# linto-ai/whisper-timestamped

Measured on NVIDIA H100. Metric: audio-sec/s (RTF) large-v3 1h synthetic @1/2/4/8 H100; DTW GB/s vs HBM peak, higher is better.
Workload: dtype bf16x3 tensor-core GEMMs (float32-accurate), f32 elsewhere, f64 DTW accumulate

## Files before the change

whisper-timestamped_b200/csrc/gemm_tc.cu:

```cuda
#include <cuda_bf16.h>

#include "sm90.cuh"

namespace wts {

constexpr int BM = 128, BN = 128, BK = 64;
constexpr int TILE_BYTES = BM * BK * 2;
constexpr int STAGES = 3;
constexpr int STAGE_BYTES = 4 * TILE_BYTES;
constexpr int PT_THREADS = 384;
constexpr int PT_PRODUCER_REGS = 40, PT_CONSUMER_REGS = 232;
static_assert(128 * PT_PRODUCER_REGS + 256 * PT_CONSUMER_REGS <= 65536, "setmaxnreg plan exceeds the register file");
constexpr int GROUP_M = 8;
constexpr int GT_SMEM = STAGES * STAGE_BYTES + 256 + 1024;
constexpr int PART_LD = BN + 4;

template <int WG>
struct SplitTraits {
    static constexpr int A_BYTES = 64 * WG * BK * 2;
    static constexpr int STAGE_BYTES = 2 * A_BYTES + 2 * TILE_BYTES;
    static constexpr int STAGES = WG == 1 ? 4 : 3;
    static constexpr int THREADS = 128 * WG + 32;
    static_assert(STAGES * STAGE_BYTES + 256 + 1024 == GT_SMEM, "a 192 KB ring: the persistent kernel's shared memory");
    static_assert(64 * WG * PART_LD * 4 <= STAGES * STAGE_BYTES, "the partial tile lives in the operand ring");
};

__device__ __forceinline__ float gelu_erf_tc(float v) { return 0.5f * v * (1.0f + erff(v * 0.70710678118654752440f)); }

struct TcArgs {
    WtsGemm g;
    int a_has_bo, a_has_bi, b_has_bo, b_has_bi;
    int split_k;
    int pair_stores;
};

__device__ __forceinline__ int64_t out_offset(const WtsGemm& g, int m, int n, int64_t ld)
{
    return g.head_dim > 0 ? (int64_t)(n / g.head_dim) * g.head_stride + (int64_t)m * ld + (n % g.head_dim)
                          : (int64_t)m * ld + n;
}

__device__ __forceinline__ void store_one(const WtsGemm& g, int m, int n, float t, float* of, __nv_bfloat16* ob)
{
    if (of) of[out_offset(g, m, n, g.ldc)] = t;
    if (ob) {
        const __nv_bfloat16 hi = __float2bfloat16_rn(t);
        __nv_bfloat16* d = ob + out_offset(g, m, n, g.ldo);
        d[0] = hi;
        d[g.o_plane] = __float2bfloat16_rn(t - __bfloat162float(hi));
    }
}

__device__ __forceinline__ float2 pair_values(const WtsGemm& g, int n, bool two, float v0, float v1, float bias_m, const float* res)
{
    float t0 = g.alpha * v0, t1 = g.alpha * v1;
    if (g.bias) {
        t0 += g.bias_on_m ? bias_m : g.bias[n];
        if (two) t1 += g.bias_on_m ? bias_m : g.bias[n + 1];
    }
    if (g.act == 1) { t0 = gelu_erf_tc(t0); t1 = gelu_erf_tc(t1); }
    if (res) { t0 += res[n]; if (two) t1 += res[n + 1]; }
    return make_float2(t0, t1);
}

__device__ __forceinline__ void store_pair_sb16(__nv_bfloat16* dh, int64_t plane, float t0, float t1)
{
    const __nv_bfloat162 hi = __floats2bfloat162_rn(t0, t1);
    const __nv_bfloat162 lo = __floats2bfloat162_rn(t0 - __low2float(hi), t1 - __high2float(hi));
    *reinterpret_cast<__nv_bfloat162*>(dh) = hi;
    *reinterpret_cast<__nv_bfloat162*>(dh + plane) = lo;
}

__device__ __forceinline__ void epilogue_pair(const WtsGemm& g, int m, int n, float v0, float v1, float bias_m,
                                              const float* res, float* of, __nv_bfloat16* ob)
{
    const bool two = n + 1 < g.N;
    const float2 t = pair_values(g, n, two, v0, v1, bias_m, res);
    const float t0 = t.x, t1 = t.y;
    const bool same_head = g.head_dim == 0 || (n % g.head_dim) + 1 < g.head_dim;
    if (!(two && same_head)) {
        store_one(g, m, n, t0, of, ob);
        if (two) store_one(g, m, n + 1, t1, of, ob);
        return;
    }
    if (of) {
        float* d = of + out_offset(g, m, n, g.ldc);
        if ((reinterpret_cast<uintptr_t>(d) & 7) == 0) *reinterpret_cast<float2*>(d) = make_float2(t0, t1);
        else { d[0] = t0; d[1] = t1; }
    }
    if (ob) {
        __nv_bfloat16* dh = ob + out_offset(g, m, n, g.ldo);
        __nv_bfloat16* dl = dh + g.o_plane;
        if (((reinterpret_cast<uintptr_t>(dh) | reinterpret_cast<uintptr_t>(dl)) & 3) == 0) {
            store_pair_sb16(dh, g.o_plane, t0, t1);
        } else {
            const __nv_bfloat162 hi = __floats2bfloat162_rn(t0, t1);
            const __nv_bfloat162 lo = __floats2bfloat162_rn(t0 - __low2float(hi), t1 - __high2float(hi));
            dh[0] = hi.x; dh[1] = hi.y; dl[0] = lo.x; dl[1] = lo.y;
        }
    }
}

template <bool PAIRS>
__device__ __forceinline__ void epilogue_frag64(const WtsGemm& g, int zo, int zi, int m_base, int n0, const float (&acc)[64])
{
    const int lane = threadIdx.x & 31;
    const int cl = 2 * (lane & 3);
    float* of = g.out_f32 ? g.out_f32 + (int64_t)zo * g.c_bo + (int64_t)zi * g.c_bi : nullptr;
    __nv_bfloat16* ob = g.out_sb16 ? reinterpret_cast<__nv_bfloat16*>(g.out_sb16) + (int64_t)zo * g.o_bo + (int64_t)zi * g.o_bi : nullptr;
#pragma unroll
    for (int i = 0; i < 2; ++i) {
        const int m = m_base + (lane >> 2) + 8 * i;
        if (m >= g.M || (g.row_mask && g.row_mask[m] == 0)) continue;
        const float* res = g.residual ? g.residual + (int64_t)zo * g.r_bo + (int64_t)zi * g.r_bi + (int64_t)m * g.ldr : nullptr;
        const float bias_m = (g.bias && g.bias_on_m) ? g.bias[m] : 0.f;
#pragma unroll
        for (int j = 0; j < 16; ++j) {
            const int n = n0 + cl + 8 * j;
            if (PAIRS) {
                const float2 t = pair_values(g, n, true, acc[4 * j + 2 * i], acc[4 * j + 2 * i + 1], bias_m, res);
                if (of) *reinterpret_cast<float2*>(of + out_offset(g, m, n, g.ldc)) = t;
                if (ob) store_pair_sb16(ob + out_offset(g, m, n, g.ldo), g.o_plane, t.x, t.y);
            } else if (n < g.N) {
                epilogue_pair(g, m, n, acc[4 * j + 2 * i], acc[4 * j + 2 * i + 1], bias_m, res, of, ob);
            }
        }
    }
}

__device__ __forceinline__ void split_epilogue_one(const WtsGemm& g, int m, int n, const float (&x)[8], float bias_n)
{
    float t = 0.f;
#pragma unroll
    for (int s = 0; s < 8; ++s) t += x[s];
    t = g.alpha * t + (g.bias ? (g.bias_on_m ? g.bias[m] : bias_n) : 0.f);
    if (g.act == 1) t = gelu_erf_tc(t);
    if (g.residual) t += g.residual[(int64_t)m * g.ldr + n];
    store_one(g, m, n, t, g.out_f32, reinterpret_cast<__nv_bfloat16*>(g.out_sb16));
}

__device__ __forceinline__ void named_bar_sync(int id, int n) { asm volatile("bar.sync %0, %1;" ::"r"(id), "r"(n) : "memory"); }
__device__ __forceinline__ void named_bar_arrive(int id, int n) { asm volatile("bar.arrive %0, %1;" ::"r"(id), "r"(n) : "memory"); }

struct TileCoord { int m0, n0, zo, zi; };

__device__ __forceinline__ TileCoord tile_coord(const WtsGemm& g, int t, int tiles_m, int tiles_n)
{
    const int per_batch = tiles_m * tiles_n;
    const int z = t / per_batch;
    int r = t - z * per_batch;
    const int span = GROUP_M * tiles_n;
    const int grp = r / span;
    const int m_first = grp * GROUP_M;
    const int gm = min(GROUP_M, tiles_m - m_first);
    r -= grp * span;
    TileCoord c;
    c.m0 = (m_first + r % gm) * BM;
    c.n0 = (r / gm) * BN;
    c.zo = z / g.batch_inner;
    c.zi = z - c.zo * g.batch_inner;
    return c;
}

__global__ void __launch_bounds__(PT_THREADS, 1)
gemm_tc_kernel(const __grid_constant__ CUtensorMap tmA, const __grid_constant__ CUtensorMap tmB, const TcArgs args)
{
    extern __shared__ unsigned char smem_raw[];
    const WtsGemm& g = args.g;
    const uint32_t base = (smem_addr(smem_raw) + 1023u) & ~1023u;
    const uint32_t bar = base + STAGES * STAGE_BYTES;
    const int wg = threadIdx.x >> 7, warp = (threadIdx.x >> 5) & 3, lane = threadIdx.x & 31;
    const int tiles_n = (g.N + BN - 1) / BN, tiles_m = (g.M + BM - 1) / BM;
    const int tiles = tiles_m * tiles_n * g.batch_outer * g.batch_inner;
    const int nkb = (g.K + BK - 1) / BK;
    pdl_launch();

    if (threadIdx.x == 0) {
        asm volatile("prefetch.tensormap [%0];" ::"l"(&tmA) : "memory");
        asm volatile("prefetch.tensormap [%0];" ::"l"(&tmB) : "memory");
        for (int s = 0; s < STAGES; ++s) { mbar_init(bar + 8 * s, 1); mbar_init(bar + 32 + 8 * s, 4); }
        asm volatile("fence.mbarrier_init.release.cluster;" ::: "memory");
    }
    __syncthreads();
    pdl_wait();

    if (wg == 0) {
        asm volatile("setmaxnreg.dec.sync.aligned.u32 %0;" ::"n"(PT_PRODUCER_REGS));
        if (warp == 0 && lane == 0) {
            int p = 0;
            for (int t = blockIdx.x; t < tiles; t += gridDim.x) {
                const TileCoord tc = tile_coord(g, t, tiles_m, tiles_n);
                const int azo = args.a_has_bo ? tc.zo : 0, azi = args.a_has_bi ? tc.zi : 0;
                const int bzo = args.b_has_bo ? tc.zo : 0, bzi = args.b_has_bi ? tc.zi : 0;
                for (int kb = 0; kb < nkb; ++kb, ++p) {
                    const int s = p % STAGES, u = p / STAGES;
                    mbar_wait(bar + 32 + 8 * s, (u & 1) ^ 1);
                    const uint32_t full = bar + 8 * s;
                    mbar_expect_tx(full, STAGE_BYTES);
                    const uint32_t st = base + s * STAGE_BYTES;
                    const int kc = kb * BK;
                    tma_load_5d(st, &tmA, full, kc, tc.m0, azi, azo, 0);
                    tma_load_5d(st + TILE_BYTES, &tmA, full, kc, tc.m0, azi, azo, 1);
                    tma_load_5d(st + 2 * TILE_BYTES, &tmB, full, kc, tc.n0, bzi, bzo, 0);
                    tma_load_5d(st + 3 * TILE_BYTES, &tmB, full, kc, tc.n0, bzi, bzo, 1);
                }
            }
        }
        return;
    }

    asm volatile("setmaxnreg.inc.sync.aligned.u32 %0;" ::"n"(PT_CONSUMER_REGS));
    const int c = wg - 1;
    float acc[2][64];
    int l = c;
    for (int t = blockIdx.x + c * gridDim.x; t < tiles; t += 2 * gridDim.x, l += 2) {
        if (l > 0) named_bar_sync(1 + c, 256);
#pragma unroll
        for (int h = 0; h < 2; ++h)
#pragma unroll
            for (int i = 0; i < 64; ++i) acc[h][i] = 0.f;
        int p = l * nkb;
        for (int kb = 0; kb < nkb; ++kb, ++p) {
            const int s = p % STAGES;
            mbar_wait(bar + 8 * s, (p / STAGES) & 1);
            const uint32_t st = base + s * STAGE_BYTES;
            const uint64_t a_hi = wg_desc(st), a_lo = wg_desc(st + TILE_BYTES);
            const uint64_t b_hi = wg_desc(st + 2 * TILE_BYTES), b_lo = wg_desc(st + 3 * TILE_BYTES);
            constexpr uint64_t a_half = (TILE_BYTES / 2) >> 4;
            wg_fence();
#pragma unroll
            for (int k = 0; k < BK / 16; ++k) {
                const uint64_t adv = (uint64_t)(k * 2);
#pragma unroll
                for (int h = 0; h < 2; ++h) wgmma_ss_n128(acc[h], a_hi + h * a_half + adv, b_hi + adv, 1);
#pragma unroll
                for (int h = 0; h < 2; ++h) wgmma_ss_n128(acc[h], a_lo + h * a_half + adv, b_hi + adv, 1);
#pragma unroll
                for (int h = 0; h < 2; ++h) wgmma_ss_n128(acc[h], a_hi + h * a_half + adv, b_lo + adv, 1);
            }
            wg_commit();
            wg_wait<1>();
            if (kb > 0 && lane == 0) mbar_arrive(bar + 32 + 8 * ((p - 1) % STAGES));
        }
        if (t + gridDim.x < tiles) named_bar_arrive(2 - c, 256);
        wg_wait<0>();
        if (lane == 0) mbar_arrive(bar + 32 + 8 * ((p - 1) % STAGES));

        const TileCoord tc = tile_coord(g, t, tiles_m, tiles_n);
        const bool pairs = args.pair_stores && tc.n0 + BN <= g.N;
#pragma unroll 1
        for (int h = 0; h < 2; ++h) {
            float v[64];
#pragma unroll
            for (int i = 0; i < 64; ++i) v[i] = h ? acc[1][i] : acc[0][i];
            if (pairs) epilogue_frag64<true>(g, tc.zo, tc.zi, tc.m0 + 64 * h + 16 * warp, tc.n0, v);
            else epilogue_frag64<false>(g, tc.zo, tc.zi, tc.m0 + 64 * h + 16 * warp, tc.n0, v);
        }
    }
}

template <int WG>
__global__ void __launch_bounds__(SplitTraits<WG>::THREADS, 1)
gemm_tc_split_kernel(const __grid_constant__ CUtensorMap tmA, const __grid_constant__ CUtensorMap tmB, const TcArgs args)
{
    using T = SplitTraits<WG>;
    extern __shared__ unsigned char smem_raw[];
    const WtsGemm& g = args.g;
    const uint32_t base = (smem_addr(smem_raw) + 1023u) & ~1023u;
    const uint32_t bar = base + T::STAGES * T::STAGE_BYTES;
    const int warp = threadIdx.x >> 5, lane = threadIdx.x & 31;
    const int n0 = blockIdx.x * BN;
    const int S = args.split_k;
    const int nkb_all = (g.K + BK - 1) / BK;
    const int kb0 = (int)((int64_t)blockIdx.z * nkb_all / S);
    const int nkb = (int)((int64_t)(blockIdx.z + 1) * nkb_all / S) - kb0;
    pdl_launch();

    if (threadIdx.x == 128 * WG) {
        asm volatile("prefetch.tensormap [%0];" ::"l"(&tmA) : "memory");
        asm volatile("prefetch.tensormap [%0];" ::"l"(&tmB) : "memory");
        for (int s = 0; s < T::STAGES; ++s) { mbar_init(bar + 8 * s, 1); mbar_init(bar + 32 + 8 * s, 4 * WG); }
        asm volatile("fence.mbarrier_init.release.cluster;" ::: "memory");
    }
    __syncthreads();

    float acc[64];
    if (warp == 4 * WG) {
        if (lane == 0) {
            const int pre = g.b_const ? min(nkb, T::STAGES) : 0;
            for (int kb = 0; kb < pre; ++kb) {
                const uint32_t st = base + kb * T::STAGE_BYTES, full = bar + 8 * kb;
                mbar_expect_tx(full, T::STAGE_BYTES);
                tma_load_5d(st + 2 * T::A_BYTES, &tmB, full, (kb0 + kb) * BK, n0, 0, 0, 0);
                tma_load_5d(st + 2 * T::A_BYTES + TILE_BYTES, &tmB, full, (kb0 + kb) * BK, n0, 0, 0, 1);
            }
            pdl_wait();
            for (int kb = 0; kb < pre; ++kb) {
                const uint32_t st = base + kb * T::STAGE_BYTES, full = bar + 8 * kb;
                tma_load_5d(st, &tmA, full, (kb0 + kb) * BK, 0, 0, 0, 0);
                tma_load_5d(st + T::A_BYTES, &tmA, full, (kb0 + kb) * BK, 0, 0, 0, 1);
            }
            for (int kb = pre; kb < nkb; ++kb) {
                const int s = kb % T::STAGES, u = kb / T::STAGES;
                mbar_wait(bar + 32 + 8 * s, (u & 1) ^ 1);
                const uint32_t full = bar + 8 * s;
                mbar_expect_tx(full, T::STAGE_BYTES);
                const uint32_t st = base + s * T::STAGE_BYTES;
                const int kc = (kb0 + kb) * BK;
                tma_load_5d(st, &tmA, full, kc, 0, 0, 0, 0);
                tma_load_5d(st + T::A_BYTES, &tmA, full, kc, 0, 0, 0, 1);
                tma_load_5d(st + 2 * T::A_BYTES, &tmB, full, kc, n0, 0, 0, 0);
                tma_load_5d(st + 2 * T::A_BYTES + TILE_BYTES, &tmB, full, kc, n0, 0, 0, 1);
            }
        } else {
            pdl_wait();
        }
    } else {
        pdl_wait();
        const uint32_t a_rows = (WG == 1 ? 0 : warp >> 2) * (T::A_BYTES / WG);
#pragma unroll
        for (int i = 0; i < 64; ++i) acc[i] = 0.f;
        for (int kb = 0; kb < nkb; ++kb) {
            const int s = kb % T::STAGES, u = kb / T::STAGES;
            mbar_wait(bar + 8 * s, u & 1);
            const uint32_t st = base + s * T::STAGE_BYTES;
            const uint64_t a_hi = wg_desc(st + a_rows), a_lo = wg_desc(st + T::A_BYTES + a_rows);
            const uint64_t b_hi = wg_desc(st + 2 * T::A_BYTES), b_lo = wg_desc(st + 2 * T::A_BYTES + TILE_BYTES);
            wg_fence();
#pragma unroll
            for (int k = 0; k < BK / 16; ++k) {
                const uint64_t adv = (uint64_t)(k * 2);
                wgmma_ss_n128(acc, a_hi + adv, b_hi + adv, 1);
                wgmma_ss_n128(acc, a_lo + adv, b_hi + adv, 1);
                wgmma_ss_n128(acc, a_hi + adv, b_lo + adv, 1);
            }
            wg_commit();
            wg_wait<1>();
            if (kb > 0 && lane == 0) mbar_arrive(bar + 32 + 8 * ((kb - 1) % T::STAGES));
        }
        wg_wait<0>();

        if (S == 1) {
            epilogue_frag64<false>(g, 0, 0, 16 * warp, n0, acc);
        } else {
            asm volatile("bar.sync 1, %0;" ::"n"(128 * WG) : "memory");
            float* part = reinterpret_cast<float*>(smem_raw + (base - smem_addr(smem_raw)));
            const int rl = 16 * warp + (lane >> 2), cl = 2 * (lane & 3);
#pragma unroll
            for (int i = 0; i < 2; ++i)
#pragma unroll
                for (int j = 0; j < 16; ++j)
                    *reinterpret_cast<float2*>(part + (rl + 8 * i) * PART_LD + cl + 8 * j) =
                        make_float2(acc[4 * j + 2 * i], acc[4 * j + 2 * i + 1]);
        }
    }
    if (S > 1) {
        __syncwarp();
        cluster_sync_all();
        if (threadIdx.x < 128 * WG) {
            uint32_t rank;
            asm volatile("mov.u32 %0, %%cluster_ctarank;" : "=r"(rank));
            const int c = 4 * lane, n = n0 + c;
            if (n < g.N) {
                uint32_t peer[8];
#pragma unroll
                for (int s = 0; s < 8; ++s) {
                    peer[s] = 0;
                    if (s < S) asm volatile("mapa.shared::cluster.u32 %0, %1, %2;" : "=r"(peer[s]) : "r"(base + 4u * c), "r"(s));
                }
                float bias_n[4];
#pragma unroll
                for (int e = 0; e < 4; ++e) bias_n[e] = (g.bias && !g.bias_on_m && n + e < g.N) ? g.bias[n + e] : 0.f;
#pragma unroll 1
                for (int m = (int)rank + S * warp; m < g.M; m += 4 * WG * S) {
                    if (g.row_mask && g.row_mask[m] == 0) continue;
                    float x[4][8];
#pragma unroll
                    for (int s = 0; s < 8; ++s) {
                        float4 v = make_float4(0.f, 0.f, 0.f, 0.f);
                        if (s < S)
                            asm volatile("ld.shared::cluster.v4.f32 {%0, %1, %2, %3}, [%4];"
                                         : "=f"(v.x), "=f"(v.y), "=f"(v.z), "=f"(v.w)
                                         : "r"(peer[s] + (uint32_t)(m * PART_LD * 4)));
                        x[0][s] = v.x; x[1][s] = v.y; x[2][s] = v.z; x[3][s] = v.w;
                    }
#pragma unroll
                    for (int e = 0; e < 4; ++e)
                        if (n + e < g.N) split_epilogue_one(g, m, n + e, x[e], bias_n[e]);
                }
            }
        }
        __syncwarp();
        cluster_sync_all();
    }
}

static int make_map(CUtensorMap* tm, const void* ptr, int64_t K, int64_t rows, int64_t ld, int64_t plane, int64_t n_bi,
                    int64_t s_bi, int64_t n_bo, int64_t s_bo, int box_rows, const char* which)
{
    auto enc = tensor_map_encoder();
    if (!enc) { set_error("wts_gemm: cuTensorMapEncodeTiled entry point not available"); return -4; }
    if ((reinterpret_cast<uintptr_t>(ptr) & 15) || (ld & 7) || (plane & 7) || (s_bi & 7) || (s_bo & 7)) {
        set_error("wts_gemm(tc): operand %s not 16-byte aligned (ptr=%p ld=%lld plane=%lld bi=%lld bo=%lld)", which, ptr,
                  (long long)ld, (long long)plane, (long long)s_bi, (long long)s_bo);
        return -5;
    }
    const int64_t e_bi = s_bi ? n_bi : 1, e_bo = s_bo ? n_bo : 1;
    cuuint64_t dims[5] = {(cuuint64_t)K, (cuuint64_t)rows, (cuuint64_t)e_bi, (cuuint64_t)e_bo, 2};
    const cuuint64_t row_b = (cuuint64_t)ld * 2;
    cuuint64_t strides[4] = {row_b, (cuuint64_t)(s_bi ? s_bi * 2 : row_b), (cuuint64_t)(s_bo ? s_bo * 2 : row_b),
                             (cuuint64_t)plane * 2};
    cuuint32_t box[5] = {BK, (cuuint32_t)box_rows, 1, 1, 1};
    cuuint32_t estr[5] = {1, 1, 1, 1, 1};
    CUresult r = enc(tm, CU_TENSOR_MAP_DATA_TYPE_BFLOAT16, 5, const_cast<void*>(ptr), dims, strides, box, estr,
                     CU_TENSOR_MAP_INTERLEAVE_NONE, CU_TENSOR_MAP_SWIZZLE_128B, CU_TENSOR_MAP_L2_PROMOTION_L2_256B,
                     CU_TENSOR_MAP_FLOAT_OOB_FILL_NONE);
    if (r != CUDA_SUCCESS) {
        set_error("wts_gemm(tc): cuTensorMapEncodeTiled(%s) failed with %d (K=%lld rows=%lld ld=%lld plane=%lld)", which, (int)r,
                  (long long)K, (long long)rows, (long long)ld, (long long)plane);
        return -6;
    }
    return 0;
}

int gemm_tc_launch(const WtsGemm& g, cudaStream_t st)
{
    static int n_sm = 0;
    if (n_sm == 0) {
        for (auto kernel : {gemm_tc_kernel, gemm_tc_split_kernel<1>, gemm_tc_split_kernel<2>})
            WTS_CUDA_CHECK(cudaFuncSetAttribute(kernel, cudaFuncAttributeMaxDynamicSharedMemorySize, GT_SMEM));
        int dev = 0;
        WTS_CUDA_CHECK(cudaGetDevice(&dev));
        WTS_CUDA_CHECK(cudaDeviceGetAttribute(&n_sm, cudaDevAttrMultiProcessorCount, dev));
    }
    const int tiles_n = (g.N + BN - 1) / BN, tiles_m = (g.M + BM - 1) / BM, nkb = (g.K + BK - 1) / BK;
    const int batch = g.batch_outer * g.batch_inner;
    const bool skinny = tiles_m == 1 && batch == 1 && g.head_dim == 0;
    const int wg = g.M <= 64 ? 1 : 2;
    alignas(64) CUtensorMap tmA, tmB;
    int rc = make_map(&tmA, g.a, g.K, g.M, g.lda, g.a_plane, g.batch_inner, g.a_bi, g.batch_outer, g.a_bo,
                      skinny ? 64 * wg : BM, "A");
    if (rc) return rc;
    rc = make_map(&tmB, g.b, g.K, g.N, g.ldb, g.b_plane, g.batch_inner, g.b_bi, g.batch_outer, g.b_bo, BN, "B");
    if (rc) return rc;
    TcArgs args;
    args.g = g;
    args.a_has_bo = g.a_bo != 0; args.a_has_bi = g.a_bi != 0;
    args.b_has_bo = g.b_bo != 0; args.b_has_bi = g.b_bi != 0;
    cudaLaunchConfig_t cfg = {};
    cfg.dynamicSmemBytes = GT_SMEM;
    cfg.stream = st;
    if (!skinny) {
        const int64_t tiles = (int64_t)tiles_m * tiles_n * batch;
        if (tiles > INT32_MAX / 2) { set_error("wts_gemm(tc): %lld output tiles are too many", (long long)tiles); return -7; }
        args.split_k = 1;
        const bool heads_even = g.head_dim == 0 || (g.head_dim % 2 == 0 && g.head_stride % 2 == 0);
        const bool of_pairs = !g.out_f32 || ((reinterpret_cast<uintptr_t>(g.out_f32) & 7) == 0 && g.ldc % 2 == 0 &&
                                             g.c_bo % 2 == 0 && g.c_bi % 2 == 0);
        const bool ob_pairs = !g.out_sb16 || ((reinterpret_cast<uintptr_t>(g.out_sb16) & 3) == 0 && g.ldo % 2 == 0 &&
                                              g.o_plane % 2 == 0 && g.o_bo % 2 == 0 && g.o_bi % 2 == 0);
        args.pair_stores = !g.row_mask && heads_even && of_pairs && ob_pairs;
        cfg.gridDim = dim3((unsigned)(tiles < n_sm ? tiles : n_sm), 1, 1);
        cfg.blockDim = dim3(PT_THREADS, 1, 1);
        WTS_CUDA_CHECK(cudaLaunchKernelEx(&cfg, gemm_tc_kernel, tmA, tmB, args));
        return 0;
    }
    int split = 1;
    if (2 * tiles_n <= n_sm) {
        split = n_sm / tiles_n;
        if (split > 8) split = 8;
        if (split > nkb) split = nkb;
    }
    args.split_k = split;
    args.pair_stores = 0;
    cfg.gridDim = dim3(tiles_n, 1, split);
    cfg.blockDim = dim3(wg == 1 ? SplitTraits<1>::THREADS : SplitTraits<2>::THREADS, 1, 1);
    cudaLaunchAttribute attr[2];
    int na = 0;
    if (split > 1) {
        attr[na].id = cudaLaunchAttributeClusterDimension;
        attr[na].val.clusterDim.x = 1;
        attr[na].val.clusterDim.y = 1;
        attr[na].val.clusterDim.z = split;
        ++na;
    }
    if (pdl_enabled()) {
        attr[na].id = cudaLaunchAttributeProgrammaticStreamSerialization;
        attr[na].val.programmaticStreamSerializationAllowed = 1;
        ++na;
    }
    cfg.attrs = attr;
    cfg.numAttrs = na;
    WTS_CUDA_CHECK(cudaLaunchKernelEx(&cfg, wg == 1 ? gemm_tc_split_kernel<1> : gemm_tc_split_kernel<2>, tmA, tmB, args));
    return 0;
}

}
```

whisper-timestamped_b200/csrc/sm90.cuh:

```cuda
#pragma once
#include <cuda.h>
#include <cudaTypedefs.h>

#include <mutex>

#include "common.cuh"

namespace wts {

__device__ __forceinline__ uint32_t smem_addr(const void* p) { return (uint32_t)__cvta_generic_to_shared(p); }

__device__ __forceinline__ void mbar_init(uint32_t bar, uint32_t count)
{
    asm volatile("mbarrier.init.shared::cta.b64 [%0], %1;" ::"r"(bar), "r"(count));
}
__device__ __forceinline__ void mbar_expect_tx(uint32_t bar, uint32_t bytes)
{
    asm volatile("mbarrier.arrive.expect_tx.shared::cta.b64 _, [%0], %1;" ::"r"(bar), "r"(bytes) : "memory");
}
__device__ __forceinline__ void mbar_arrive(uint32_t bar)
{
    asm volatile("mbarrier.arrive.shared::cta.b64 _, [%0];" ::"r"(bar) : "memory");
}
__device__ __forceinline__ void mbar_wait(uint32_t bar, uint32_t parity)
{
    asm volatile(
        "{\n\t"
        ".reg .pred p;\n\t"
        "WAIT_LOOP:\n\t"
        "mbarrier.try_wait.parity.shared::cta.b64 p, [%0], %1;\n\t"
        "@p bra DONE;\n\t"
        "bra WAIT_LOOP;\n\t"
        "DONE:\n\t"
        "}\n" ::"r"(bar), "r"(parity) : "memory");
}
__device__ __forceinline__ void tma_load_4d(uint32_t dst, const CUtensorMap* tm, uint32_t bar, int c0, int c1, int c2, int c3)
{
    asm volatile(
        "cp.async.bulk.tensor.4d.shared::cluster.global.mbarrier::complete_tx::bytes [%0], [%1, {%3, %4, %5, %6}], [%2];"
        ::"r"(dst), "l"(tm), "r"(bar), "r"(c0), "r"(c1), "r"(c2), "r"(c3) : "memory");
}
__device__ __forceinline__ void tma_load_5d(uint32_t dst, const CUtensorMap* tm, uint32_t bar, int c0, int c1, int c2,
                                            int c3, int c4)
{
    asm volatile(
        "cp.async.bulk.tensor.5d.shared::cluster.global.mbarrier::complete_tx::bytes [%0], [%1, {%3, %4, %5, %6, %7}], [%2];"
        ::"r"(dst), "l"(tm), "r"(bar), "r"(c0), "r"(c1), "r"(c2), "r"(c3), "r"(c4) : "memory");
}

__device__ __forceinline__ uint64_t wg_desc(uint32_t saddr)
{
    uint64_t d = 0;
    d |= (uint64_t)((saddr >> 4) & 0x3FFF);
    d |= (uint64_t)1 << 16;
    d |= (uint64_t)(1024 >> 4) << 32;
    d |= (uint64_t)1 << 62;
    return d;
}
__device__ __forceinline__ void wg_fence() { asm volatile("wgmma.fence.sync.aligned;" ::: "memory"); }
__device__ __forceinline__ void wg_commit() { asm volatile("wgmma.commit_group.sync.aligned;" ::: "memory"); }
template <int N> __device__ __forceinline__ void wg_wait() { asm volatile("wgmma.wait_group.sync.aligned %0;" ::"n"(N) : "memory"); }

__device__ __forceinline__ void wgmma_ss_n128(float (&d)[64], uint64_t a, uint64_t b, int scale_d)
{
    asm volatile(
        "{\n\t.reg .pred p;\n\tsetp.ne.b32 p, %66, 0;\n\t"
        "wgmma.mma_async.sync.aligned.m64n128k16.f32.bf16.bf16 {%0, %1, %2, %3, %4, %5, %6, %7, %8, %9, %10, %11, %12, %13, %14, %15, %16, %17, %18, %19, %20, %21, %22, %23, %24, %25, %26, %27, %28, %29, %30, %31, %32, %33, %34, %35, %36, %37, %38, %39, %40, %41, %42, %43, %44, %45, %46, %47, %48, %49, %50, %51, %52, %53, %54, %55, %56, %57, %58, %59, %60, %61, %62, %63}, %64, %65, p, 1, 1, 0, 0;\n\t}\n"
        : "+f"(d[0]), "+f"(d[1]), "+f"(d[2]), "+f"(d[3]), "+f"(d[4]), "+f"(d[5]), "+f"(d[6]), "+f"(d[7]), "+f"(d[8]), "+f"(d[9]), "+f"(d[10]), "+f"(d[11]), "+f"(d[12]), "+f"(d[13]), "+f"(d[14]), "+f"(d[15]), "+f"(d[16]), "+f"(d[17]), "+f"(d[18]), "+f"(d[19]), "+f"(d[20]), "+f"(d[21]), "+f"(d[22]), "+f"(d[23]), "+f"(d[24]), "+f"(d[25]), "+f"(d[26]), "+f"(d[27]), "+f"(d[28]), "+f"(d[29]), "+f"(d[30]), "+f"(d[31]), "+f"(d[32]), "+f"(d[33]), "+f"(d[34]), "+f"(d[35]), "+f"(d[36]), "+f"(d[37]), "+f"(d[38]), "+f"(d[39]), "+f"(d[40]), "+f"(d[41]), "+f"(d[42]), "+f"(d[43]), "+f"(d[44]), "+f"(d[45]), "+f"(d[46]), "+f"(d[47]), "+f"(d[48]), "+f"(d[49]), "+f"(d[50]), "+f"(d[51]), "+f"(d[52]), "+f"(d[53]), "+f"(d[54]), "+f"(d[55]), "+f"(d[56]), "+f"(d[57]), "+f"(d[58]), "+f"(d[59]), "+f"(d[60]), "+f"(d[61]), "+f"(d[62]), "+f"(d[63])
        : "l"(a), "l"(b), "r"(scale_d));
}

__device__ __forceinline__ void wgmma_rs_n64(float (&d)[32], const uint32_t* a, uint64_t b)
{
    asm volatile(
        "{\n\t.reg .pred p;\n\tsetp.ne.b32 p, %37, 0;\n\t"
        "wgmma.mma_async.sync.aligned.m64n64k16.f32.bf16.bf16 {%0, %1, %2, %3, %4, %5, %6, %7, %8, %9, %10, %11, %12, %13, %14, %15, %16, %17, %18, %19, %20, %21, %22, %23, %24, %25, %26, %27, %28, %29, %30, %31}, {%32, %33, %34, %35}, %36, p, 1, 1, 0;\n\t}\n"
        : "+f"(d[0]), "+f"(d[1]), "+f"(d[2]), "+f"(d[3]), "+f"(d[4]), "+f"(d[5]), "+f"(d[6]), "+f"(d[7]), "+f"(d[8]), "+f"(d[9]), "+f"(d[10]), "+f"(d[11]), "+f"(d[12]), "+f"(d[13]), "+f"(d[14]), "+f"(d[15]), "+f"(d[16]), "+f"(d[17]), "+f"(d[18]), "+f"(d[19]), "+f"(d[20]), "+f"(d[21]), "+f"(d[22]), "+f"(d[23]), "+f"(d[24]), "+f"(d[25]), "+f"(d[26]), "+f"(d[27]), "+f"(d[28]), "+f"(d[29]), "+f"(d[30]), "+f"(d[31])
        : "r"(a[0]), "r"(a[1]), "r"(a[2]), "r"(a[3]), "l"(b), "r"(1));
}

__device__ __forceinline__ void cluster_sync_all()
{
    asm volatile("barrier.cluster.arrive.release.aligned;" ::: "memory");
    asm volatile("barrier.cluster.wait.acquire.aligned;" ::: "memory");
}

inline PFN_cuTensorMapEncodeTiled_v12000 tensor_map_encoder()
{
    static PFN_cuTensorMapEncodeTiled_v12000 fn = nullptr;
    static std::once_flag once;
    std::call_once(once, [] {
        void* p = nullptr;
        cudaDriverEntryPointQueryResult qres;
        if (cudaGetDriverEntryPoint("cuTensorMapEncodeTiled", &p, cudaEnableDefault, &qres) == cudaSuccess &&
            qres == cudaDriverEntryPointSuccess)
            fn = reinterpret_cast<PFN_cuTensorMapEncodeTiled_v12000>(p);
    });
    return fn;
}

}
```

Measured before the change: 641.9.

## Pair persistent GEMM CTAs into 2-CTA clusters with TMA multicast of shared operand

The persistent bf16x3 GEMM now runs as 2-CTA clusters. Each cluster processes a pair of adjacent output tiles that share either the A or the B operand. Each CTA loads half of the shared operand and multicasts it to both CTAs, which is meant to cut L2/HBM operand traffic per tile. The empty barriers now count arrivals from consumers in both CTAs, and producers drain the ring before exiting. In exchange, the cluster couples the progress of paired CTAs and may cut the number of resident CTAs when the tile count is odd.

```diff
diff --git a/whisper-timestamped_b200/csrc/gemm_tc.cu b/whisper-timestamped_b200/csrc/gemm_tc.cu
--- a/whisper-timestamped_b200/csrc/gemm_tc.cu
+++ b/whisper-timestamped_b200/csrc/gemm_tc.cu
@@ -12,6 +12,7 @@
 constexpr int PT_PRODUCER_REGS = 40, PT_CONSUMER_REGS = 232;
 static_assert(128 * PT_PRODUCER_REGS + 256 * PT_CONSUMER_REGS <= 65536, "setmaxnreg plan exceeds the register file");
 constexpr int GROUP_M = 8;
+constexpr int HALF_BYTES = TILE_BYTES / 2;
 constexpr int GT_SMEM = STAGES * STAGE_BYTES + 256 + 1024;
 constexpr int PART_LD = BN + 4;
 
@@ -32,6 +33,7 @@
     int a_has_bo, a_has_bi, b_has_bo, b_has_bi;
     int split_k;
     int pair_stores;
+    int pair_n;
 };
 
 __device__ __forceinline__ int64_t out_offset(const WtsGemm& g, int m, int n, int64_t ld)
@@ -144,19 +146,21 @@
 
 struct TileCoord { int m0, n0, zo, zi; };
 
-__device__ __forceinline__ TileCoord tile_coord(const WtsGemm& g, int t, int tiles_m, int tiles_n)
-{
-    const int per_batch = tiles_m * tiles_n;
-    const int z = t / per_batch;
-    int r = t - z * per_batch;
-    const int span = GROUP_M * tiles_n;
+__device__ __forceinline__ TileCoord pair_coord(const WtsGemm& g, int q, int pm, int pn, bool pair_n, int rank)
+{
+    const int per_batch = pm * pn;
+    const int z = q / per_batch;
+    int r = q - z * per_batch;
+    const int gsz = pair_n ? GROUP_M : GROUP_M / 2;
+    const int span = gsz * pn;
     const int grp = r / span;
-    const int m_first = grp * GROUP_M;
-    const int gm = min(GROUP_M, tiles_m - m_first);
+    const int m_first = grp * gsz;
+    const int gm = min(gsz, pm - m_first);
     r -= grp * span;
+    const int mi = m_first + r % gm, ni = r / gm;
     TileCoord c;
-    c.m0 = (m_first + r % gm) * BM;
-    c.n0 = (r / gm) * BN;
+    c.m0 = (pair_n ? mi : 2 * mi + rank) * BM;
+    c.n0 = (pair_n ? 2 * ni + rank : ni) * BN;
     c.zo = z / g.batch_inner;
     c.zi = z - c.zo * g.batch_inner;
     return c;
@@ -171,25 +175,28 @@
     const uint32_t bar = base + STAGES * STAGE_BYTES;
     const int wg = threadIdx.x >> 7, warp = (threadIdx.x >> 5) & 3, lane = threadIdx.x & 31;
     const int tiles_n = (g.N + BN - 1) / BN, tiles_m = (g.M + BM - 1) / BM;
-    const int tiles = tiles_m * tiles_n * g.batch_outer * g.batch_inner;
+    const bool pair_n = args.pair_n;
+    const int pm = pair_n ? tiles_m : (tiles_m + 1) / 2, pn = pair_n ? (tiles_n + 1) / 2 : tiles_n;
+    const int n_pairs = pm * pn * g.batch_outer * g.batch_inner;
     const int nkb = (g.K + BK - 1) / BK;
+    const int rank = (int)cluster_ctarank(), cluster = blockIdx.x >> 1, clusters = gridDim.x >> 1;
     pdl_launch();
 
     if (threadIdx.x == 0) {
         asm volatile("prefetch.tensormap [%0];" ::"l"(&tmA) : "memory");
         asm volatile("prefetch.tensormap [%0];" ::"l"(&tmB) : "memory");
-        for (int s = 0; s < STAGES; ++s) { mbar_init(bar + 8 * s, 1); mbar_init(bar + 32 + 8 * s, 4); }
+        for (int s = 0; s < STAGES; ++s) { mbar_init(bar + 8 * s, 1); mbar_init(bar + 32 + 8 * s, 8); }
         asm volatile("fence.mbarrier_init.release.cluster;" ::: "memory");
     }
-    __syncthreads();
+    cluster_sync_all();
     pdl_wait();
 
     if (wg == 0) {
         asm volatile("setmaxnreg.dec.sync.aligned.u32 %0;" ::"n"(PT_PRODUCER_REGS));
         if (warp == 0 && lane == 0) {
             int p = 0;
-            for (int t = blockIdx.x; t < tiles; t += gridDim.x) {
-                const TileCoord tc = tile_coord(g, t, tiles_m, tiles_n);
+            for (int q = cluster; q < n_pairs; q += clusters) {
+                const TileCoord tc = pair_coord(g, q, pm, pn, pair_n, rank);
                 const int azo = args.a_has_bo ? tc.zo : 0, azi = args.a_has_bi ? tc.zi : 0;
                 const int bzo = args.b_has_bo ? tc.zo : 0, bzi = args.b_has_bi ? tc.zi : 0;
                 for (int kb = 0; kb < nkb; ++kb, ++p) {
@@ -199,12 +206,22 @@
                     mbar_expect_tx(full, STAGE_BYTES);
                     const uint32_t st = base + s * STAGE_BYTES;
                     const int kc = kb * BK;
-                    tma_load_5d(st, &tmA, full, kc, tc.m0, azi, azo, 0);
-                    tma_load_5d(st + TILE_BYTES, &tmA, full, kc, tc.m0, azi, azo, 1);
-                    tma_load_5d(st + 2 * TILE_BYTES, &tmB, full, kc, tc.n0, bzi, bzo, 0);
-                    tma_load_5d(st + 3 * TILE_BYTES, &tmB, full, kc, tc.n0, bzi, bzo, 1);
+                    if (pair_n) {
+                        const int m = tc.m0 + 64 * rank;
+                        tma_load_5d_multicast(st + rank * HALF_BYTES, &tmA, full, 3, kc, m, azi, azo, 0);
+                        tma_load_5d_multicast(st + TILE_BYTES + rank * HALF_BYTES, &tmA, full, 3, kc, m, azi, azo, 1);
+                        tma_load_5d(st + 2 * TILE_BYTES, &tmB, full, kc, tc.n0, bzi, bzo, 0);
+                        tma_load_5d(st + 3 * TILE_BYTES, &tmB, full, kc, tc.n0, bzi, bzo, 1);
+                    } else {
+                        const int n = tc.n0 + 64 * rank;
+                        tma_load_5d(st, &tmA, full, kc, tc.m0, azi, azo, 0);
+                        tma_load_5d(st + TILE_BYTES, &tmA, full, kc, tc.m0, azi, azo, 1);
+                        tma_load_5d_multicast(st + 2 * TILE_BYTES + rank * HALF_BYTES, &tmB, full, 3, kc, n, bzi, bzo, 0);
+                        tma_load_5d_multicast(st + 3 * TILE_BYTES + rank * HALF_BYTES, &tmB, full, 3, kc, n, bzi, bzo, 1);
+                    }
                 }
             }
+            for (int i = 0; i < STAGES; ++i, ++p) mbar_wait(bar + 32 + 8 * (p % STAGES), ((p / STAGES) & 1) ^ 1);
         }
         return;
     }
@@ -212,8 +229,8 @@
     asm volatile("setmaxnreg.inc.sync.aligned.u32 %0;" ::"n"(PT_CONSUMER_REGS));
     const int c = wg - 1;
     float acc[2][64];
-    int l = c;
-    for (int t = blockIdx.x + c * gridDim.x; t < tiles; t += 2 * gridDim.x, l += 2) {
+    for (int q = cluster + c * clusters; q < n_pairs; q += 2 * clusters) {
+        const int l = (q - cluster) / clusters;
         if (l > 0) named_bar_sync(1 + c, 256);
 #pragma unroll
         for (int h = 0; h < 2; ++h)
@@ -240,13 +257,19 @@
             }
             wg_commit();
             wg_wait<1>();
-            if (kb > 0 && lane == 0) mbar_arrive(bar + 32 + 8 * ((p - 1) % STAGES));
-        }
-        if (t + gridDim.x < tiles) named_bar_arrive(2 - c, 256);
+            if (kb > 0 && lane == 0) {
+                mbar_arrive_cluster(bar + 32 + 8 * ((p - 1) % STAGES), 0);
+                mbar_arrive_cluster(bar + 32 + 8 * ((p - 1) % STAGES), 1);
+            }
+        }
+        if (q + clusters < n_pairs) named_bar_arrive(2 - c, 256);
         wg_wait<0>();
-        if (lane == 0) mbar_arrive(bar + 32 + 8 * ((p - 1) % STAGES));
-
-        const TileCoord tc = tile_coord(g, t, tiles_m, tiles_n);
+        if (lane == 0) {
+            mbar_arrive_cluster(bar + 32 + 8 * ((p - 1) % STAGES), 0);
+            mbar_arrive_cluster(bar + 32 + 8 * ((p - 1) % STAGES), 1);
+        }
+
+        const TileCoord tc = pair_coord(g, q, pm, pn, pair_n, rank);
         const bool pairs = args.pair_stores && tc.n0 + BN <= g.N;
 #pragma unroll 1
         for (int h = 0; h < 2; ++h) {
@@ -425,23 +448,38 @@
 
 int gemm_tc_launch(const WtsGemm& g, cudaStream_t st)
 {
-    static int n_sm = 0;
+    static int n_sm = 0, n_clusters = 0;
     if (n_sm == 0) {
         for (auto kernel : {gemm_tc_kernel, gemm_tc_split_kernel<1>, gemm_tc_split_kernel<2>})
             WTS_CUDA_CHECK(cudaFuncSetAttribute(kernel, cudaFuncAttributeMaxDynamicSharedMemorySize, GT_SMEM));
         int dev = 0;
         WTS_CUDA_CHECK(cudaGetDevice(&dev));
         WTS_CUDA_CHECK(cudaDeviceGetAttribute(&n_sm, cudaDevAttrMultiProcessorCount, dev));
+        cudaLaunchConfig_t occ = {};
+        cudaLaunchAttribute ca;
+        ca.id = cudaLaunchAttributeClusterDimension;
+        ca.val.clusterDim.x = 2;
+        ca.val.clusterDim.y = 1;
+        ca.val.clusterDim.z = 1;
+        occ.gridDim = dim3(2 * n_sm, 1, 1);
+        occ.blockDim = dim3(PT_THREADS, 1, 1);
+        occ.dynamicSmemBytes = GT_SMEM;
+        occ.attrs = &ca;
+        occ.numAttrs = 1;
+        WTS_CUDA_CHECK(cudaOccupancyMaxActiveClusters(&n_clusters, gemm_tc_kernel, &occ));
+        if (n_clusters < 1) { set_error("wts_gemm(tc): no 2-CTA cluster of the persistent GEMM fits on this device"); n_sm = 0; return -8; }
     }
     const int tiles_n = (g.N + BN - 1) / BN, tiles_m = (g.M + BM - 1) / BM, nkb = (g.K + BK - 1) / BK;
     const int batch = g.batch_outer * g.batch_inner;
     const bool skinny = tiles_m == 1 && batch == 1 && g.head_dim == 0;
     const int wg = g.M <= 64 ? 1 : 2;
+    const bool pair_n = tiles_m % 2 == 1 && (tiles_n % 2 == 0 || tiles_m <= tiles_n);
     alignas(64) CUtensorMap tmA, tmB;
     int rc = make_map(&tmA, g.a, g.K, g.M, g.lda, g.a_plane, g.batch_inner, g.a_bi, g.batch_outer, g.a_bo,
-                      skinny ? 64 * wg : BM, "A");
+                      skinny ? 64 * wg : (pair_n ? BM / 2 : BM), "A");
     if (rc) return rc;
-    rc = make_map(&tmB, g.b, g.K, g.N, g.ldb, g.b_plane, g.batch_inner, g.b_bi, g.batch_outer, g.b_bo, BN, "B");
+    rc = make_map(&tmB, g.b, g.K, g.N, g.ldb, g.b_plane, g.batch_inner, g.b_bi, g.batch_outer, g.b_bo,
+                  skinny || pair_n ? BN : BN / 2, "B");
     if (rc) return rc;
     TcArgs args;
     args.g = g;
@@ -451,17 +489,25 @@
     cfg.dynamicSmemBytes = GT_SMEM;
     cfg.stream = st;
     if (!skinny) {
-        const int64_t tiles = (int64_t)tiles_m * tiles_n * batch;
-        if (tiles > INT32_MAX / 2) { set_error("wts_gemm(tc): %lld output tiles are too many", (long long)tiles); return -7; }
+        const int64_t pairs = (int64_t)(pair_n ? tiles_m : (tiles_m + 1) / 2) * (pair_n ? (tiles_n + 1) / 2 : tiles_n) * batch;
+        if (pairs > INT32_MAX / 2) { set_error("wts_gemm(tc): %lld output tile pairs are too many", (long long)pairs); return -7; }
         args.split_k = 1;
+        args.pair_n = pair_n;
         const bool heads_even = g.head_dim == 0 || (g.head_dim % 2 == 0 && g.head_stride % 2 == 0);
         const bool of_pairs = !g.out_f32 || ((reinterpret_cast<uintptr_t>(g.out_f32) & 7) == 0 && g.ldc % 2 == 0 &&
                                              g.c_bo % 2 == 0 && g.c_bi % 2 == 0);
         const bool ob_pairs = !g.out_sb16 || ((reinterpret_cast<uintptr_t>(g.out_sb16) & 3) == 0 && g.ldo % 2 == 0 &&
                                               g.o_plane % 2 == 0 && g.o_bo % 2 == 0 && g.o_bi % 2 == 0);
         args.pair_stores = !g.row_mask && heads_even && of_pairs && ob_pairs;
-        cfg.gridDim = dim3((unsigned)(tiles < n_sm ? tiles : n_sm), 1, 1);
+        cfg.gridDim = dim3(2 * (unsigned)(pairs < n_clusters ? pairs : n_clusters), 1, 1);
         cfg.blockDim = dim3(PT_THREADS, 1, 1);
+        cudaLaunchAttribute ca;
+        ca.id = cudaLaunchAttributeClusterDimension;
+        ca.val.clusterDim.x = 2;
+        ca.val.clusterDim.y = 1;
+        ca.val.clusterDim.z = 1;
+        cfg.attrs = &ca;
+        cfg.numAttrs = 1;
         WTS_CUDA_CHECK(cudaLaunchKernelEx(&cfg, gemm_tc_kernel, tmA, tmB, args));
         return 0;
     }
@@ -473,6 +519,7 @@
     }
     args.split_k = split;
     args.pair_stores = 0;
+    args.pair_n = 0;
     cfg.gridDim = dim3(tiles_n, 1, split);
     cfg.blockDim = dim3(wg == 1 ? SplitTraits<1>::THREADS : SplitTraits<2>::THREADS, 1, 1);
     cudaLaunchAttribute attr[2];
diff --git a/whisper-timestamped_b200/csrc/sm90.cuh b/whisper-timestamped_b200/csrc/sm90.cuh
--- a/whisper-timestamped_b200/csrc/sm90.cuh
+++ b/whisper-timestamped_b200/csrc/sm90.cuh
@@ -46,6 +46,28 @@
     asm volatile(
         "cp.async.bulk.tensor.5d.shared::cluster.global.mbarrier::complete_tx::bytes [%0], [%1, {%3, %4, %5, %6, %7}], [%2];"
         ::"r"(dst), "l"(tm), "r"(bar), "r"(c0), "r"(c1), "r"(c2), "r"(c3), "r"(c4) : "memory");
+}
+__device__ __forceinline__ void tma_load_5d_multicast(uint32_t dst, const CUtensorMap* tm, uint32_t bar, uint16_t cta_mask,
+                                                      int c0, int c1, int c2, int c3, int c4)
+{
+    asm volatile(
+        "cp.async.bulk.tensor.5d.shared::cluster.global.mbarrier::complete_tx::bytes.multicast::cluster"
+        " [%0], [%1, {%4, %5, %6, %7, %8}], [%2], %3;"
+        ::"r"(dst), "l"(tm), "r"(bar), "h"(cta_mask), "r"(c0), "r"(c1), "r"(c2), "r"(c3), "r"(c4) : "memory");
+}
+
+__device__ __forceinline__ uint32_t cluster_ctarank()
+{
+    uint32_t r;
+    asm volatile("mov.u32 %0, %%cluster_ctarank;" : "=r"(r));
+    return r;
+}
+
+__device__ __forceinline__ void mbar_arrive_cluster(uint32_t bar, uint32_t cta)
+{
+    uint32_t remote;
+    asm volatile("mapa.shared::cluster.u32 %0, %1, %2;" : "=r"(remote) : "r"(bar), "r"(cta));
+    asm volatile("mbarrier.arrive.shared::cluster.b64 _, [%0];" ::"r"(remote) : "memory");
 }
 
 __device__ __forceinline__ uint64_t wg_desc(uint32_t saddr)
```

Result: no change. 642.5 (median of 6 runs) (+0.1%).
